# dryajov/zkinterface-ir

Hardware: NVIDIA B200
Metric: field gates evaluated/sec (higher is better)
Workload: dtype u32x8 (255-bit field, Montgomery)

## Files before the change

### zkinterface-ir_b200/csrc/kernels.cu

```cuda
#include <cuda_runtime.h>
#include <stdint.h>
#include <stdlib.h>
#include <string.h>

#include <cooperative_groups.h>

#include "device_util.cuh"
#include "kernels.cuh"

namespace cg = cooperative_groups;

namespace zkb {

template <int N>
__global__ void k_to_mont(uint32_t* consts, uint32_t n, FieldParams fp) {
    uint32_t i = blockIdx.x * blockDim.x + threadIdx.x;
    if (i >= n) return;
    uint32_t a[N], r[N];
#pragma unroll
    for (int k = 0; k < N; k++) a[k] = consts[(size_t)i * N + k];
    fe_mont_mul<N>(r, a, fp.r2, fp.p, fp.n0inv);
#pragma unroll
    for (int k = 0; k < N; k++) consts[(size_t)i * N + k] = r[k];
}
// ... 119 lines not shown
}

template <int N, bool RARE>
__global__ void __launch_bounds__(256)
k_level(const GateOp* __restrict__ ops, const uint32_t* __restrict__ aseq, uint64_t n_ops, uint32_t* __restrict__ store,
        const uint32_t* __restrict__ consts_mont, uint32_t* __restrict__ first_fail, RawCtx rc, TileGeom g, FieldParams fp) {
    const uint64_t total = n_ops << g.log2_wt;
    const uint32_t wt_mask = (1u << g.log2_wt) - 1;
    const bool single = g.log2_wt == 0;
    for (uint64_t tid = blockIdx.x * (uint64_t)blockDim.x + threadIdx.x; tid < total;
         tid += (uint64_t)gridDim.x * blockDim.x) {
        const uint32_t lane = (uint32_t)tid & wt_mask;
        const uint64_t gi = tid >> g.log2_wt;
        const uint4 raw = __ldg(reinterpret_cast<const uint4*>(ops) + gi);
        const uint32_t opc = raw.w & 0xff;
        uint32_t a[N], b[N], r[N];
        load_elem<N>(a, store, raw.x, lane, g.log2_wt);
        if (!RARE) {
            if (opc == D_ADDC || opc == D_MULC) {
#pragma unroll
                for (int k = 0; k < N; k++) b[k] = __ldg(consts_mont + (size_t)raw.y * N + k);
            } else {
                load_elem<N>(b, store, raw.y, lane, g.log2_wt);
            }
            if (opc == D_ADD || opc == D_ADDC) fe_add<N>(r, a, b, fp.p);
            else fe_mont_mul<N>(r, a, b, fp.p, fp.n0inv);
        } else {
            if (opc == D_AND || opc == D_XOR) {
                load_elem<N>(b, store, raw.y, lane, g.log2_wt);
            } else {
#pragma unroll
                for (int k = 0; k < N; k++) b[k] = 0;
            }
            rare_gate<N>(r, a, b, raw, lane, g, rc, fp);
        }
        if (!(raw.w & (F_NOSTORE | g.skip_mask))) store_elem<N>(store, raw.z, lane, g.log2_wt, r);
        if (raw.w & F_ASSERT) {
            bool fail = !fe_is_zero<N>(r) && lane < g.n_valid;
            report_fail(fail, __ldg(aseq + gi), first_fail, g.batch0 + lane, single);
        }
    }
}

template <int N, int LPT>
__device__ __forceinline__ void load_operands(uint32_t* a, uint32_t* b, const uint4& d, const uint32_t* __restrict__ store,
                                              const uint32_t* __restrict__ consts_mont, uint32_t plane, uint32_t log2_pwt) {
    constexpr int PN = N * LPT;
    const uint32_t opc = d.w & 0xff;
    load_elem<PN>(a, store, d.x, plane, log2_pwt);
    if (opc == D_ADDC || opc == D_MULC) {
#pragma unroll
        for (int l = 0; l < LPT; l++)
#pragma unroll
            for (int k = 0; k < N; k++) b[l * N + k] = __ldg(consts_mont + (size_t)d.y * N + k);
    } else {
        load_elem<PN>(b, store, d.y, plane, log2_pwt);
    }
}

#ifndef ZKB_LEVEL_PIPE_MIN_CTAS
#define ZKB_LEVEL_PIPE_MIN_CTAS 4
#endif
template <int N, int LPT>
__global__ void __launch_bounds__(256, ZKB_LEVEL_PIPE_MIN_CTAS)
k_level_pipe(const GateOp* __restrict__ ops, const uint32_t* __restrict__ aseq, uint64_t n_ops, uint32_t* __restrict__ store,
             const uint32_t* __restrict__ consts_mont, uint32_t* __restrict__ first_fail, TileGeom g, FieldParams fp) {
    constexpr int PN = N * LPT;
    constexpr uint32_t kLog2Lpt = LPT == 4 ? 2 : LPT == 2 ? 1 : 0;
    const uint32_t log2_pwt = g.log2_wt - kLog2Lpt;
    const uint64_t total = n_ops << log2_pwt;
    const uint32_t pwt_mask = (1u << log2_pwt) - 1;
    const bool single = g.log2_wt == 0;
    const uint64_t stride = (uint64_t)gridDim.x * blockDim.x;
    uint64_t t0 = blockIdx.x * (uint64_t)blockDim.x + threadIdx.x;
    if (t0 >= total) return;
    const uint4* dptr = reinterpret_cast<const uint4*>(ops);
    uint64_t t1 = t0 + stride, t2 = t1 + stride;
    uint4 d0 = __ldg(dptr + (t0 >> log2_pwt));
    uint4 d1 = t1 < total ? __ldg(dptr + (t1 >> log2_pwt)) : make_uint4(0, 0, 0, 0);
    uint32_t a0[PN], b0[PN], a1[PN], b1[PN];
    load_operands<N, LPT>(a0, b0, d0, store, consts_mont, (uint32_t)t0 & pwt_mask, log2_pwt);
    while (true) {
        uint4 d2 = make_uint4(0, 0, 0, 0);
        if (t2 < total) d2 = __ldg(dptr + (t2 >> log2_pwt));
        const bool more = t1 < total;
        if (more) load_operands<N, LPT>(a1, b1, d1, store, consts_mont, (uint32_t)t1 & pwt_mask, log2_pwt);
        const uint32_t opc = d0.w & 0xff;
        const uint32_t plane = (uint32_t)t0 & pwt_mask;
        uint32_t r[PN];
#pragma unroll
        for (int l = 0; l < LPT; l++) {
            if (opc == D_ADD || opc == D_ADDC) fe_add<N>(r + l * N, a0 + l * N, b0 + l * N, fp.p);
            else fe_mont_mul<N>(r + l * N, a0 + l * N, b0 + l * N, fp.p, fp.n0inv);
        }
        if (!(d0.w & (F_NOSTORE | g.skip_mask))) store_elem<PN>(store, d0.z, plane, log2_pwt, r);
        if (d0.w & F_ASSERT) {
            const uint32_t seq = __ldg(aseq + (t0 >> log2_pwt));
#pragma unroll
            for (int l = 0; l < LPT; l++) {
                const uint32_t lane = plane * LPT + l;
                bool fail = !fe_is_zero<N>(r + l * N) && lane < g.n_valid;
                report_fail(fail, seq, first_fail, g.batch0 + lane, single);
            }
        }
        if (!more) break;
#pragma unroll
        for (int k = 0; k < PN; k++) {
            a0[k] = a1[k];
            b0[k] = b1[k];
        }
        d0 = d1;
        d1 = d2;
        t0 = t1;
        t1 = t2;
        t2 += stride;
    }
}

#ifndef ZKB_TMA_STAGES
#define ZKB_TMA_STAGES 3
#endif
#ifndef ZKB_TMA_MIN_CTAS
#define ZKB_TMA_MIN_CTAS 4
#endif
__device__ __forceinline__ void mbar_init(uint32_t bar, uint32_t count) {
    asm volatile("mbarrier.init.shared::cta.b64 [%0], %1;" ::"r"(bar), "r"(count) : "memory");
}
__device__ __forceinline__ void mbar_expect_tx(uint32_t bar, uint32_t bytes) {
    asm volatile("mbarrier.arrive.expect_tx.shared::cta.b64 _, [%0], %1;" ::"r"(bar), "r"(bytes) : "memory");
}
__device__ __forceinline__ void mbar_wait(uint32_t bar, uint32_t parity) {
    asm volatile(
        "{\n"
        ".reg .pred p;\n"
        "WAIT_%=:\n"
        "mbarrier.try_wait.parity.shared::cta.b64 p, [%0], %1;\n"
        "@p bra DONE_%=;\n"
        "bra WAIT_%=;\n"
        "DONE_%=:\n"
        "}\n" ::"r"(bar), "r"(parity) : "memory");
}
__device__ __forceinline__ void bulk_g2s(uint32_t dst, const void* src, uint32_t bytes, uint32_t bar) {
    asm volatile("cp.async.bulk.shared::cluster.global.mbarrier::complete_tx::bytes [%0], [%1], %2, [%3];" ::"r"(dst), "l"(src), "r"(bytes),
                 "r"(bar)
                 : "memory");
}
__device__ __forceinline__ uint4 lds128(uint32_t a) {
    uint4 v;
    asm volatile("ld.shared.v4.u32 {%0, %1, %2, %3}, [%4];" : "=r"(v.x), "=r"(v.y), "=r"(v.z), "=r"(v.w) : "r"(a));
    return v;
}

constexpr size_t kTmaSmemBytes = (size_t)ZKB_TMA_STAGES * 16384;

template <int N>
__global__ void __launch_bounds__(256, ZKB_TMA_MIN_CTAS)
k_level_tma(const GateOp* __restrict__ ops, const uint32_t* __restrict__ aseq, uint64_t n_ops, uint32_t* __restrict__ store,
            const uint32_t* __restrict__ consts_mont, uint32_t* __restrict__ first_fail, TileGeom g, FieldParams fp) {
    static_assert(N == 8, "two 16-byte chunks per element");
    constexpr int S = ZKB_TMA_STAGES;
    constexpr uint32_t ELEM = 8192, STAGE = 2 * ELEM;
    extern __shared__ __align__(128) uint8_t tma_smem[];
    __shared__ __align__(8) uint64_t full_bar[S];
    const uint32_t smem0 = (uint32_t)__cvta_generic_to_shared(tma_smem);
    const uint32_t bar0 = (uint32_t)__cvta_generic_to_shared(full_bar);
    const uint4* dptr = reinterpret_cast<const uint4*>(ops);
    const uint8_t* store_b = reinterpret_cast<const uint8_t*>(store);
    const uint32_t log2_q = g.log2_wt - 8;
    const uint32_t q_mask = (1u << log2_q) - 1;
    const uint64_t n_items = n_ops << log2_q;
    const uint32_t row = 4096u << log2_q;
    const uint64_t stride = gridDim.x;
    uint64_t gi = blockIdx.x;
    if (gi >= n_items) return;
    auto issue = [&](uint32_t stage, const uint4& d, uint32_t q) {
        const uint32_t opc = d.w & 0xff;
        const bool two = !(opc == D_ADDC || opc == D_MULC);
        const uint32_t bar = bar0 + stage * 8;
        mbar_expect_tx(bar, two ? STAGE : ELEM);
        const uint8_t* pa = store_b + (size_t)d.x * 2 * row + (size_t)q * 4096;
        bulk_g2s(smem0 + stage * STAGE, pa, 4096, bar);
        bulk_g2s(smem0 + stage * STAGE + 4096, pa + row, 4096, bar);
        if (two) {
            const uint8_t* pb = store_b + (size_t)d.y * 2 * row + (size_t)q * 4096;
            bulk_g2s(smem0 + stage * STAGE + ELEM, pb, 4096, bar);
            bulk_g2s(smem0 + stage * STAGE + ELEM + 4096, pb + row, 4096, bar);
        }
    };
    uint64_t gp = gi;
    uint4 dp = make_uint4(0, 0, 0, 0);
    if (threadIdx.x == 0) {
#pragma unroll
        for (int i = 0; i < S; i++) mbar_init(bar0 + i * 8, 1);
        asm volatile("fence.mbarrier_init.release.cluster;" ::: "memory");
        asm volatile("fence.proxy.async.shared::cta;" ::: "memory");
#pragma unroll
        for (int i = 0; i < S; i++) {
            if (gp < n_items) issue(i, __ldg(dptr + (gp >> log2_q)), (uint32_t)gp & q_mask);
            gp += stride;
        }
        if (gp < n_items) dp = __ldg(dptr + (gp >> log2_q));
    }
    __syncthreads();
    uint4 d0 = __ldg(dptr + (gi >> log2_q));
    for (uint32_t it = 0;; it++) {
        const uint64_t gn = gi + stride;
        uint4 d1 = make_uint4(0, 0, 0, 0);
        if (gn < n_items) d1 = __ldg(dptr + (gn >> log2_q));
        const uint32_t lane = (((uint32_t)gi & q_mask) << 8) + threadIdx.x;
        const uint32_t stage = it % S, parity = (it / S) & 1;
        const uint32_t opc = d0.w & 0xff;
        uint32_t a[N], b[N], r[N];
        mbar_wait(bar0 + stage * 8, parity);
        const uint32_t sa = smem0 + stage * STAGE + threadIdx.x * 16;
        unpack(lds128(sa), a);
        unpack(lds128(sa + 4096), a + 4);
        if (opc == D_ADDC || opc == D_MULC) {
#pragma unroll
            for (int k = 0; k < N; k++) b[k] = __ldg(consts_mont + (size_t)d0.y * N + k);
        } else {
            unpack(lds128(sa + ELEM), b);
            unpack(lds128(sa + ELEM + 4096), b + 4);
        }
        __syncthreads();
        if (threadIdx.x == 0) {
            if (gp < n_items) {
                issue(stage, dp, (uint32_t)gp & q_mask);
                gp += stride;
                if (gp < n_items) dp = __ldg(dptr + (gp >> log2_q));
            }
        }
        if (opc == D_ADD || opc == D_ADDC) fe_add<N>(r, a, b, fp.p);
        else fe_mont_mul<N>(r, a, b, fp.p, fp.n0inv);
        if (!(d0.w & (F_NOSTORE | g.skip_mask))) store_elem<N>(store, d0.z, lane, g.log2_wt, r);
        if (d0.w & F_ASSERT) {
            const uint32_t seq = __ldg(aseq + (gi >> log2_q));
            bool fail = !fe_is_zero<N>(r) && lane < g.n_valid;
            report_fail(fail, seq, first_fail, g.batch0 + lane, false);
        }
        if (gn >= n_items) break;
        d0 = d1;
        gi = gn;
    }
}

__device__ __forceinline__ void grid_barrier(uint32_t* ctr, uint32_t target) {
    __syncthreads();
    if (threadIdx.x == 0) {
        asm volatile("red.release.gpu.global.add.u32 [%0], 1;" ::"l"(ctr) : "memory");
        uint32_t v;
        do {
            asm volatile("ld.relaxed.gpu.global.u32 %0, [%1];" : "=r"(v) : "l"(ctr) : "memory");
        } while ((int32_t)(v - target) < 0);
        asm volatile("fence.acq_rel.gpu;" ::: "memory");
    }
    __syncthreads();
}

#ifdef ZKB_COOP_PROFILE
__device__ __forceinline__ long long zkb_clock() {
    long long t;
    asm volatile("mov.u64 %0, %%clock64;" : "=l"(t)::"memory");
    return t;
}
#endif
__device__ __forceinline__ uint4 ldg_pinned(const uint4* p) {
    uint4 v;
    asm volatile("ld.global.nc.v4.u32 {%0, %1, %2, %3}, [%4];" : "=r"(v.x), "=r"(v.y), "=r"(v.z), "=r"(v.w) : "l"(p));
    return v;
}

template <int N, bool CLUSTER>
__global__ void __launch_bounds__(CLUSTER ? 512 : 256)
k_levels_coop(const GateOp* __restrict__ ops, const uint32_t* __restrict__ aseq, const uint64_t* __restrict__ level_off,
              uint32_t n_levels, uint32_t* store, const uint32_t* __restrict__ consts_mont, uint32_t* __restrict__ first_fail,
              RawCtx rc, TileGeom g, FieldParams fp, uint32_t* barrier_ctr, uint32_t barrier_base) {
    const uint32_t wt_mask = (1u << g.log2_wt) - 1;
    const bool single = g.log2_wt == 0;
    const uint64_t stride = (uint64_t)gridDim.x * blockDim.x;
    const uint64_t tid0 = blockIdx.x * (uint64_t)blockDim.x + threadIdx.x;
    const uint4* dptr = reinterpret_cast<const uint4*>(ops);
    constexpr uint32_t kOffCache = 2048;
    __shared__ uint64_t s_off[kOffCache + 1];
    for (uint32_t i = threadIdx.x; i <= n_levels && i <= kOffCache; i += blockDim.x) s_off[i] = level_off[i];
    __syncthreads();
    auto off = [&](uint32_t i) -> uint64_t { return i <= kOffCache ? s_off[i] : level_off[i]; };
    uint64_t lo = off(0), hi = n_levels ? off(1) : lo;
    uint4 first = make_uint4(0, 0, 0, 0);
    if (tid0 < ((hi - lo) << g.log2_wt)) first = ldg_pinned(dptr + lo + (tid0 >> g.log2_wt));
#ifdef ZKB_COOP_PROFILE
    long long prof[7] = {0, 0, 0, 0, 0, 0, 0};
#endif
    for (uint32_t l = 0; l < n_levels; l++) {
#ifdef ZKB_COOP_PROFILE
        const long long th0 = zkb_clock();
#endif
        const uint64_t total = (hi - lo) << g.log2_wt;
        uint64_t nlo = hi, nhi = hi;
        uint4 next_first = make_uint4(0, 0, 0, 0);
        if (l + 1 < n_levels) {
            nhi = off(l + 2);
            if (tid0 < ((nhi - nlo) << g.log2_wt)) next_first = ldg_pinned(dptr + nlo + (tid0 >> g.log2_wt));
        }
#ifdef ZKB_COOP_PROFILE
        const long long tw0 = zkb_clock();
        prof[0] += tw0 - th0;
#endif
        for (uint64_t tid = tid0; tid < total; tid += stride) {
            const uint32_t lane = (uint32_t)tid & wt_mask;
            const uint64_t gi = lo + (tid >> g.log2_wt);
            const uint4 raw = tid == tid0 ? first : __ldg(dptr + gi);
            const uint32_t opc = raw.w & 0xff;
            uint32_t a[N], b[N], r[N];
            load_elem_coherent<N>(a, store, raw.x, lane, g.log2_wt);
            if (opc == D_ADDC || opc == D_MULC) {
#pragma unroll
                for (int k = 0; k < N; k++) b[k] = __ldg(consts_mont + (size_t)raw.y * N + k);
            } else if (opc == D_ADD || opc == D_MUL || opc == D_AND || opc == D_XOR) {
                load_elem_coherent<N>(b, store, raw.y, lane, g.log2_wt);
            } else {
#pragma unroll
                for (int k = 0; k < N; k++) b[k] = 0;
            }
#ifdef ZKB_COOP_PROFILE
            long long tq0 = zkb_clock();
            prof[6] += tq0 - tw0;
            if ((a[0] ^ b[0]) == 0x12345678u) tq0++;
            const long long tq1 = zkb_clock();
            prof[3] += tq1 - tq0;
#endif
            if (opc == D_ADD || opc == D_ADDC) fe_add<N>(r, a, b, fp.p);
            else if (opc == D_MUL || opc == D_MULC) fe_mont_mul<N>(r, a, b, fp.p, fp.n0inv);
            else rare_gate<N>(r, a, b, raw, lane, g, rc, fp);
#ifdef ZKB_COOP_PROFILE
            long long tq2 = zkb_clock();
            if (r[0] == 0x12345679u) tq2++;
            prof[4] += tq2 - tq1;
#endif
            if (!(raw.w & F_NOSTORE)) store_elem<N>(store, raw.z, lane, g.log2_wt, r);
            if (raw.w & F_ASSERT) {
                bool fail = !fe_is_zero<N>(r) && lane < g.n_valid;
                report_fail(fail, __ldg(aseq + gi), first_fail, g.batch0 + lane, single);
            }
#ifdef ZKB_COOP_PROFILE
            prof[5] += zkb_clock() - tq2;
#endif
        }
#ifdef ZKB_COOP_PROFILE
        prof[1] += zkb_clock() - tw0;
#endif
        first = next_first;
        lo = nlo;
        hi = nhi;
        if (l + 1 < n_levels) {
#ifdef ZKB_COOP_PROFILE
            const long long tb0 = zkb_clock();
#endif
            if (CLUSTER) cg::this_cluster().sync();
            else if (barrier_ctr) grid_barrier(barrier_ctr, barrier_base + gridDim.x * (l + 1));
            else cg::this_grid().sync();
#ifdef ZKB_COOP_PROFILE
            prof[2] += zkb_clock() - tb0;
#endif
        }
    }
#ifdef ZKB_COOP_PROFILE
    if ((threadIdx.x & 31) == 0 && (blockIdx.x == 0 || blockIdx.x == gridDim.x - 1) && (threadIdx.x == 0 || threadIdx.x == blockDim.x - 32))
        printf("coop profile cta %u warp %u: levels %u  head %lld  work %lld (issue %lld operands %lld compute %lld store+assert %lld)  barrier %lld  (cycles per level)\n",
               blockIdx.x, threadIdx.x / 32, n_levels, prof[0] / n_levels, prof[1] / n_levels, prof[6] / n_levels, prof[3] / n_levels, prof[4] / n_levels,
               prof[5] / n_levels, prof[2] / n_levels);
#endif
}

template <int N>
__device__ __forceinline__ uint64_t flow_peek(const uint32_t* store, uint32_t slot) {
    if constexpr (N == 2) {
        uint64_t v;
        asm volatile("ld.relaxed.gpu.global.u64 %0, [%1];" : "=l"(v) : "l"(reinterpret_cast<const uint64_t*>(store) + slot) : "memory");
        return v;
    } else {
        uint32_t v;
        asm volatile("ld.relaxed.gpu.global.u32 %0, [%1];" : "=r"(v) : "l"(store + slot) : "memory");
        return v == ~0u ? ~0ull : (uint64_t)v;
    }
}
template <int N>
__device__ __forceinline__ void flow_publish_elem(uint32_t* store, uint32_t slot, const uint32_t* r) {
    if constexpr (N == 2) {
        const uint64_t v = (uint64_t)r[1] << 32 | r[0];
        asm volatile("st.relaxed.gpu.global.u64 [%0], %1;" ::"l"(reinterpret_cast<uint64_t*>(store) + slot), "l"(v) : "memory");
    } else {
        asm volatile("st.relaxed.gpu.global.u32 [%0], %1;" ::"l"(store + slot), "r"(r[0]) : "memory");
    }
}

// ... 443 lines not shown
                } else {
                    uint32_t a[N], one[N], r[N];
                    load_elem<N>(a, store, d.slot, j, g.log2_wt);
#pragma unroll
                    for (int k = 0; k < N; k++) one[k] = (k == 0);
                    fe_mont_mul<N>(r, a, one, fp.p, fp.n0inv);
#pragma unroll
                    for (int k = 0; k < N; k++) dst[k] = r[k];
                    w = N;
                }
            } else {
                const uint8_t* src;
                uint32_t len;
                if (d.kind == CAP_RAW_CONST) {
                    src = raw_consts + (size_t)d.opb * raw_stride;
                    len = raw_stride;
                } else {
                    const uint64_t widx = g.batch0 + j;
                    src = (d.kind == CAP_INSTANCE ? in.inst + widx * in.inst_set_stride : in.wit + widx * in.wit_set_stride) +
                          (uint64_t)d.opb * in.stride;
                    len = in.stride;
                }
                for (; 4 * w < len; w++) {
                    uint32_t x = 0;
                    for (uint32_t b = 0; b < 4 && 4 * w + b < len; b++) x |= (uint32_t)src[4 * w + b] << (8 * b);
                    dst[w] = x;
                }
            }
            for (; w < ew; w++) dst[w] = 0;
        }
        __syncthreads();
        const uint32_t nl = min(kCaptureLanes, g.n_valid - lb * kCaptureLanes);
        const uint32_t per_lane = nv * ew;
        for (uint32_t q = v * kCaptureLanes + l; q < nl * per_lane; q += vb * kCaptureLanes) {
            const uint32_t ll = q / per_lane, r = q - ll * per_lane;
            out[((size_t)(g.batch0 + lb * kCaptureLanes + ll) * n + i0) * ew + r] = cap_sm[ll * row + r];
        }
        __syncthreads();
    }
}

template <int N>
__global__ void __launch_bounds__(256)
k_capture(const CaptureDesc* __restrict__ descs, uint32_t n, const uint32_t* __restrict__ store, InputDesc in,
          const uint8_t* __restrict__ raw_consts, uint32_t raw_stride, TileGeom g, uint32_t ew, uint32_t* __restrict__ out, FieldParams fp) {
    capture_tile<N>(descs, n, store, in, raw_consts, raw_stride, g, ew, out, fp);
}

__global__ void __launch_bounds__(256)
k_bool_capture(const CaptureDesc* __restrict__ descs, uint32_t n, const uint32_t* __restrict__ store, InputDesc in,
               const uint8_t* __restrict__ raw_consts, uint32_t raw_stride, TileGeom g, uint32_t ew, uint32_t* __restrict__ out, FieldParams fp) {
    capture_tile<0>(descs, n, store, in, raw_consts, raw_stride, g, ew, out, fp);
}

__global__ void k_unsink(GateOp* ops, uint64_t n_ops, const uint32_t* __restrict__ slot_bits, uint32_t* found, uint32_t cap, uint32_t* n_found) {
    for (uint64_t i = blockIdx.x * (uint64_t)blockDim.x + threadIdx.x; i < n_ops; i += (uint64_t)gridDim.x * blockDim.x) {
        const uint32_t m = ops[i].meta;
        if (!(m & F_SINK)) continue;
        const uint32_t s = ops[i].out;
        if (!((slot_bits[s >> 5] >> (s & 31)) & 1)) continue;
        ops[i].meta = m & ~F_SINK;
        const uint32_t k = atomicAdd(n_found, 1u);
        if (k < cap) found[k] = (uint32_t)i;
    }
}

__global__ void k_set_sink(GateOp* ops, const uint32_t* __restrict__ idx, uint32_t n, uint32_t set) {
    const uint32_t i = blockIdx.x * blockDim.x + threadIdx.x;
    if (i >= n) return;
    GateOp& op = ops[idx[i]];
    op.meta = set ? (op.meta | F_SINK) : (op.meta & ~F_SINK);
}

__global__ void k_fill_u32(uint32_t* p, uint32_t v, uint64_t n) {
    for (uint64_t i = blockIdx.x * (uint64_t)blockDim.x + threadIdx.x; i < n; i += (uint64_t)gridDim.x * blockDim.x) p[i] = v;
}

static bool level_pipe_enabled() {
    static int v = -1;
    if (v < 0) {
        const char* e = getenv("ZKB_LEVEL_PIPE");
        v = e ? (atoi(e) != 0) : 1;
    }
    return v != 0;
}
static bool level_tma_enabled() {
    const char* e = getenv("ZKB_LEVEL_TMA");
    return e ? atoi(e) != 0 : true;
}
static int grid_per_sm(int dflt) {
    static int v = -1;
    if (v < 0) {
        const char* e = getenv("ZKB_GRID_PER_SM");
        v = e ? atoi(e) : 0;
    }
    return v > 0 ? v : dflt;
}

static inline unsigned grid_for(uint64_t total, int sm_count, int per_sm) {
    uint64_t blocks = (total + 255) / 256;
    uint64_t cap = (uint64_t)sm_count * per_sm;
    if (blocks > cap) blocks = cap;
    if (blocks == 0) blocks = 1;
    return (unsigned)blocks;
}

#define ZKB_DISPATCH_N(nlimb, CALL)         \
    switch (nlimb) {                        \
        case 1: { constexpr int N = 1; CALL; } break; \
        case 2: { constexpr int N = 2; CALL; } break; \
        case 4: { constexpr int N = 4; CALL; } break; \
        default: { constexpr int N = 8; CALL; } break; \
    }

void launch_to_mont(int nlimb, uint32_t* consts, uint32_t n, const FieldParams& fp, cudaStream_t s) {
    if (n == 0) return;
    ZKB_DISPATCH_N(nlimb, (k_to_mont<N><<<(n + 127) / 128, 128, 0, s>>>(consts, n, fp)));
}

void launch_load_inputs(int nlimb, const InputLoad* loads, uint32_t n_loads, uint32_t* store, const uint32_t* consts_mont,
                        InputDesc in, TileGeom g, uint32_t* unreduced_count, uint8_t* rawflag, const uint8_t* const_flags,
                        const FieldParams& fp, int sm_count, cudaStream_t s) {
    if (n_loads == 0) return;
    unsigned grid = grid_for((uint64_t)n_loads << g.log2_wt, sm_count, 256);
    ZKB_DISPATCH_N(nlimb, (k_load_inputs<N><<<grid, 256, 0, s>>>(loads, n_loads, store, consts_mont, in, g, unreduced_count, rawflag,
                                                                 const_flags, fp)));
}

void launch_level(int nlimb, const GateOp* ops, const uint32_t* aseq, uint64_t n_ops, uint32_t* store,
                  const uint32_t* consts_mont, uint32_t* first_fail, const RawCtx& rc, TileGeom g, const FieldParams& fp,
                  int sm_count, bool rare, cudaStream_t s) {
    if (n_ops == 0) return;
    unsigned grid = grid_for(n_ops << g.log2_wt, sm_count, grid_per_sm(256));
    if (!rare) {
        if (level_pipe_enabled()) {
            static const bool pack = getenv("ZKB_LEVEL_LPT") == nullptr || atoi(getenv("ZKB_LEVEL_LPT")) != 1;
            if (pack && nlimb == 2 && g.log2_wt >= 6) {
                grid = grid_for(n_ops << (g.log2_wt - 1), sm_count, grid_per_sm(256));
                k_level_pipe<2, 2><<<grid, 256, 0, s>>>(ops, aseq, n_ops, store, consts_mont, first_fail, g, fp);
            } else if (pack && nlimb == 1 && g.log2_wt >= 7) {
                grid = grid_for(n_ops << (g.log2_wt - 2), sm_count, grid_per_sm(256));
                k_level_pipe<1, 4><<<grid, 256, 0, s>>>(ops, aseq, n_ops, store, consts_mont, first_fail, g, fp);
            } else if (nlimb == 8 && g.log2_wt >= 8 && level_tma_enabled()) {
                static int tma_per_sm = 0;
                static std::atomic<uint64_t> tma_attr_seen{0};
                constexpr size_t smem = kTmaSmemBytes;
                if (first_on_device(tma_attr_seen))
                    cudaFuncSetAttribute(k_level_tma<8>, cudaFuncAttributeMaxDynamicSharedMemorySize, (int)smem);
                if (!tma_per_sm) {
                    const char* e = getenv("ZKB_TMA_GRID_PER_SM");
                    tma_per_sm = e ? std::max(1, atoi(e)) : 128;
                }
                grid = grid_for(n_ops << g.log2_wt, sm_count, tma_per_sm);
                k_level_tma<8><<<grid, 256, smem, s>>>(ops, aseq, n_ops, store, consts_mont, first_fail, g, fp);
            } else {
                ZKB_DISPATCH_N(nlimb, (k_level_pipe<N, 1><<<grid, 256, 0, s>>>(ops, aseq, n_ops, store, consts_mont, first_fail, g, fp)));
            }
        } else {
            ZKB_DISPATCH_N(nlimb, (k_level<N, false><<<grid, 256, 0, s>>>(ops, aseq, n_ops, store, consts_mont, first_fail, rc, g, fp)));
        }
    } else {
        ZKB_DISPATCH_N(nlimb, (k_level<N, true><<<grid, 256, 0, s>>>(ops, aseq, n_ops, store, consts_mont, first_fail, rc, g, fp)));
    }
}

template <int N>
static cudaError_t launch_coop_n(const GateOp* ops, const uint32_t* aseq, const uint64_t* level_off, uint32_t n_levels, uint32_t* store,
                                 const uint32_t* consts_mont, uint32_t* first_fail, RawCtx rc, TileGeom g, FieldParams fp,
                                 int sm_count, uint64_t max_level_items, uint32_t* barrier_ctr, uint32_t* barrier_epoch, cudaStream_t s) {
    static const bool counter_barrier = getenv("ZKB_COUNTER_BARRIER") != nullptr;
    if (!counter_barrier) barrier_ctr = nullptr;
    uint32_t barrier_base = *barrier_epoch;
    void* args[] = {(void*)&ops, (void*)&aseq, (void*)&level_off, (void*)&n_levels, (void*)&store, (void*)&consts_mont,
                    (void*)&first_fail, (void*)&rc, (void*)&g, (void*)&fp, (void*)&barrier_ctr, (void*)&barrier_base};
    static const bool no_cluster = getenv("ZKB_NO_CLUSTER") != nullptr;
    static bool cluster_ok = true;
    if (!no_cluster && cluster_ok && max_level_items <= 8 * 512 * 2) {
        cudaLaunchConfig_t cfg = {};
        cfg.gridDim = dim3(8);
        cfg.blockDim = dim3(512);
        cfg.stream = s;
        cudaLaunchAttribute attr[1];
        attr[0].id = cudaLaunchAttributeClusterDimension;
        attr[0].val.clusterDim.x = 8;
        attr[0].val.clusterDim.y = 1;
        attr[0].val.clusterDim.z = 1;
        cfg.attrs = attr;
        cfg.numAttrs = 1;
        cudaError_t ec = cudaLaunchKernelExC(&cfg, (const void*)k_levels_coop<N, true>, args);
        if (ec == cudaSuccess) return ec;
        cudaGetLastError();
        cluster_ok = false;
    }
    int per_sm = 0;
    cudaError_t e = cudaOccupancyMaxActiveBlocksPerMultiprocessor(&per_sm, k_levels_coop<N, false>, 256, 0);
    if (e != cudaSuccess) return e;
    if (per_sm < 1) return cudaErrorLaunchOutOfResources;
    uint64_t want = (max_level_items + 255) / 256;
    uint64_t blocks = ((want + sm_count - 1) / sm_count) * sm_count;
    if (blocks < (uint64_t)sm_count) blocks = sm_count;
    if (blocks > (uint64_t)sm_count * per_sm) blocks = (uint64_t)sm_count * per_sm;
    if (const char* e = getenv("ZKB_COOP_BLOCKS")) blocks = (uint64_t)atoi(e);
    e = cudaLaunchCooperativeKernel((void*)k_levels_coop<N, false>, dim3((unsigned)blocks), dim3(256), args, 0, s);
    if (e == cudaSuccess && barrier_ctr && n_levels > 1) *barrier_epoch += (uint32_t)blocks * (n_levels - 1);
    return e;
}

template <int KIND>
__global__ void __launch_bounds__(KIND == 2 ? 512 : 256) k_barrier_only(uint32_t n, uint32_t* ctr, uint32_t base, uint32_t* sink) {
    uint32_t acc = 0;
    for (uint32_t i = 0; i < n; i++) {
        if (KIND == 0) cg::this_grid().sync();
        else if (KIND == 1) grid_barrier(ctr, base + gridDim.x * (i + 1));
        else cg::this_cluster().sync();
        acc += i;
    }
    if (acc == 0xFFFFFFFFu) *sink = acc;
}

cudaError_t measure_barrier_cost(int kind, unsigned blocks, unsigned n_barriers, uint32_t* barrier_ctr, uint32_t* barrier_epoch,
                                 cudaStream_t s, cudaEvent_t ev0, cudaEvent_t ev1, float* us_per_barrier) {
    uint32_t base = *barrier_epoch;
    uint32_t* sink = barrier_ctr;
    float best = 1e30f;
    for (int rep = 0; rep < 4; rep++) {
        float ms[2] = {0, 0};
        for (int pass = 0; pass < 2; pass++) {
            uint32_t n = pass == 0 ? 0u : n_barriers;
            base = *barrier_epoch;
            void* args[] = {(void*)&n, (void*)&barrier_ctr, (void*)&base, (void*)&sink};
            cudaEventRecord(ev0, s);
            cudaError_t e;
            if (kind == 2) {
                cudaLaunchConfig_t cfg = {};
                cfg.gridDim = dim3(8);
                cfg.blockDim = dim3(512);
                cfg.stream = s;
                cudaLaunchAttribute attr[1];
                attr[0].id = cudaLaunchAttributeClusterDimension;
                attr[0].val.clusterDim.x = 8;
                attr[0].val.clusterDim.y = 1;
                attr[0].val.clusterDim.z = 1;
                cfg.attrs = attr;
                cfg.numAttrs = 1;
                e = cudaLaunchKernelExC(&cfg, (const void*)k_barrier_only<2>, args);
            } else if (kind == 1) {
                e = cudaLaunchCooperativeKernel((void*)k_barrier_only<1>, dim3(blocks), dim3(256), args, 0, s);
                if (e == cudaSuccess) *barrier_epoch += blocks * n;
            } else {
                e = cudaLaunchCooperativeKernel((void*)k_barrier_only<0>, dim3(blocks), dim3(256), args, 0, s);
            }
            if (e != cudaSuccess) return e;
            cudaEventRecord(ev1, s);
            e = cudaStreamSynchronize(s);
            if (e != cudaSuccess) return e;
            cudaEventElapsedTime(&ms[pass], ev0, ev1);
        }
        if (rep > 0) best = std::min(best, ms[1] - ms[0]);
    }
    *us_per_barrier = best * 1e3f / (float)n_barriers;
    return cudaSuccess;
}

cudaError_t launch_levels_coop(int nlimb, const GateOp* ops, const uint32_t* aseq, const uint64_t* level_off, uint32_t n_levels,
                               uint32_t* store, const uint32_t* consts_mont, uint32_t* first_fail, const RawCtx& rc, TileGeom g,
                               const FieldParams& fp, int sm_count, uint64_t max_level_items, uint32_t* barrier_ctr,
                               uint32_t* barrier_epoch, cudaStream_t s) {
    cudaError_t e = cudaSuccess;
    ZKB_DISPATCH_N(nlimb, (e = launch_coop_n<N>(ops, aseq, level_off, n_levels, store, consts_mont, first_fail, rc, g, fp, sm_count,
                                                max_level_items, barrier_ctr, barrier_epoch, s)));
    return e;
}

template <int N>
static cudaError_t launch_flow_n(const GateOp* ops, const uint32_t* aseq, const uint64_t* level_off, uint32_t n_levels, uint32_t* store,
                                 const uint32_t* consts_mont, uint32_t* first_fail, RawCtx rc, TileGeom g, FieldParams fp, int sm_count,
                                 uint64_t max_level_items, uint32_t fill_from, uint32_t n_slots, cudaStream_t s) {
    int per_sm = 0;
    cudaError_t e = cudaOccupancyMaxActiveBlocksPerMultiprocessor(&per_sm, k_levels_flow<N>, 256, 0);
    if (e != cudaSuccess) return e;
    if (per_sm < 1) return cudaErrorLaunchOutOfResources;
    uint64_t want = (max_level_items + 255) / 256;
    uint64_t blocks = ((want + sm_count - 1) / sm_count) * sm_count;
    if (blocks < (uint64_t)sm_count) blocks = sm_count;
    if (blocks > (uint64_t)sm_count * per_sm) blocks = (uint64_t)sm_count * per_sm;
    if (const char* eb = getenv("ZKB_FLOW_BLOCKS")) blocks = std::min<uint64_t>((uint64_t)std::max(1, atoi(eb)), (uint64_t)sm_count * per_sm);
    if (n_slots > fill_from) {
        e = cudaMemsetAsync(store + (size_t)fill_from * N, 0xFF, (size_t)(n_slots - fill_from) * N * 4, s);
        if (e != cudaSuccess) return e;
    }
    uint32_t sleep_ns = 0;
    if (const char* es = getenv("ZKB_FLOW_SLEEP")) sleep_ns = (uint32_t)atoi(es);
    void* args[] = {(void*)&ops, (void*)&aseq, (void*)&level_off, (void*)&n_levels, (void*)&store, (void*)&consts_mont,
                    (void*)&first_fail, (void*)&rc, (void*)&g, (void*)&fp, (void*)&sleep_ns};
    return cudaLaunchCooperativeKernel((void*)k_levels_flow<N>, dim3((unsigned)blocks), dim3(256), args, 0, s);
}
template <int N>
static cudaError_t launch_flow_wide_n(const GateOp* ops, const uint32_t* aseq, const uint64_t* level_off, uint32_t n_levels, uint32_t* store,
                                      const uint32_t* consts_mont, uint32_t* first_fail, RawCtx rc, TileGeom g, FieldParams fp, int sm_count,
                                      uint64_t max_level_items, uint32_t n_ready, uint32_t* flags, uint32_t epoch, cudaStream_t s) {
    int per_sm = 0;
    cudaError_t e = cudaOccupancyMaxActiveBlocksPerMultiprocessor(&per_sm, k_levels_flow_wide<N>, 256, 0);
    if (e != cudaSuccess) return e;
    if (per_sm < 1) return cudaErrorLaunchOutOfResources;
    uint64_t want = (max_level_items + 255) / 256;
    uint64_t blocks = ((want + sm_count - 1) / sm_count) * sm_count;
    if (blocks < (uint64_t)sm_count) blocks = sm_count;
// ... 167 lines not shown
```

Before: 77.92 billion.

## Add dedicated producer warp with empty/full mbarriers to TMA level kernel

Restructures the TMA level kernel into a warp-specialized producer/consumer pipeline: an extra warp issues bulk copies and writes op descriptors to shared memory, and consumer warps signal per-stage empty barriers instead of a block-wide __syncthreads. This removes the per-iteration block barrier and lets the refill overlap with compute. It costs an extra warp per CTA, which may cut occupancy under the launch bounds, and adds barrier traffic.

```diff
diff --git a/zkinterface-ir_b200/csrc/kernels.cu b/zkinterface-ir_b200/csrc/kernels.cu
--- a/zkinterface-ir_b200/csrc/kernels.cu
+++ b/zkinterface-ir_b200/csrc/kernels.cu
@@ -295,18 +295,28 @@
 }
 
 constexpr size_t kTmaSmemBytes = (size_t)ZKB_TMA_STAGES * 16384;
-
-template <int N>
-__global__ void __launch_bounds__(256, ZKB_TMA_MIN_CTAS)
+constexpr int kTmaThreads = 256 + 32;
+__device__ __forceinline__ void mbar_arrive(uint32_t bar) {
+    asm volatile("mbarrier.arrive.shared::cta.b64 _, [%0];" ::"r"(bar) : "memory");
+}
+__device__ __forceinline__ void sts128(uint32_t a, const uint4& v) {
+    asm volatile("st.shared.v4.u32 [%0], {%1, %2, %3, %4};" ::"r"(a), "r"(v.x), "r"(v.y), "r"(v.z), "r"(v.w) : "memory");
+}
+
+template <int N>
+__global__ void __launch_bounds__(kTmaThreads, ZKB_TMA_MIN_CTAS)
 k_level_tma(const GateOp* __restrict__ ops, const uint32_t* __restrict__ aseq, uint64_t n_ops, uint32_t* __restrict__ store,
             const uint32_t* __restrict__ consts_mont, uint32_t* __restrict__ first_fail, TileGeom g, FieldParams fp) {
     static_assert(N == 8, "two 16-byte chunks per element");
     constexpr int S = ZKB_TMA_STAGES;
     constexpr uint32_t ELEM = 8192, STAGE = 2 * ELEM;
     extern __shared__ __align__(128) uint8_t tma_smem[];
-    __shared__ __align__(8) uint64_t full_bar[S];
+    __shared__ __align__(8) uint64_t full_bar[S], empty_bar[S];
+    __shared__ __align__(16) uint4 desc[S];
     const uint32_t smem0 = (uint32_t)__cvta_generic_to_shared(tma_smem);
-    const uint32_t bar0 = (uint32_t)__cvta_generic_to_shared(full_bar);
+    const uint32_t full0 = (uint32_t)__cvta_generic_to_shared(full_bar);
+    const uint32_t empty0 = (uint32_t)__cvta_generic_to_shared(empty_bar);
+    const uint32_t desc0 = (uint32_t)__cvta_generic_to_shared(desc);
     const uint4* dptr = reinterpret_cast<const uint4*>(ops);
     const uint8_t* store_b = reinterpret_cast<const uint8_t*>(store);
     const uint32_t log2_q = g.log2_wt - 8;
@@ -314,64 +324,66 @@
     const uint64_t n_items = n_ops << log2_q;
     const uint32_t row = 4096u << log2_q;
     const uint64_t stride = gridDim.x;
-    uint64_t gi = blockIdx.x;
-    if (gi >= n_items) return;
-    auto issue = [&](uint32_t stage, const uint4& d, uint32_t q) {
-        const uint32_t opc = d.w & 0xff;
-        const bool two = !(opc == D_ADDC || opc == D_MULC);
-        const uint32_t bar = bar0 + stage * 8;
-        mbar_expect_tx(bar, two ? STAGE : ELEM);
-        const uint8_t* pa = store_b + (size_t)d.x * 2 * row + (size_t)q * 4096;
-        bulk_g2s(smem0 + stage * STAGE, pa, 4096, bar);
-        bulk_g2s(smem0 + stage * STAGE + 4096, pa + row, 4096, bar);
-        if (two) {
-            const uint8_t* pb = store_b + (size_t)d.y * 2 * row + (size_t)q * 4096;
-            bulk_g2s(smem0 + stage * STAGE + ELEM, pb, 4096, bar);
-            bulk_g2s(smem0 + stage * STAGE + ELEM + 4096, pb + row, 4096, bar);
-        }
-    };
-    uint64_t gp = gi;
-    uint4 dp = make_uint4(0, 0, 0, 0);
+    if (blockIdx.x >= n_items) return;
     if (threadIdx.x == 0) {
 #pragma unroll
-        for (int i = 0; i < S; i++) mbar_init(bar0 + i * 8, 1);
+        for (int i = 0; i < S; i++) {
+            mbar_init(full0 + i * 8, 1);
+            mbar_init(empty0 + i * 8, 256 / 32);
+        }
         asm volatile("fence.mbarrier_init.release.cluster;" ::: "memory");
         asm volatile("fence.proxy.async.shared::cta;" ::: "memory");
-#pragma unroll
-        for (int i = 0; i < S; i++) {
-            if (gp < n_items) issue(i, __ldg(dptr + (gp >> log2_q)), (uint32_t)gp & q_mask);
-            gp += stride;
-        }
-        if (gp < n_items) dp = __ldg(dptr + (gp >> log2_q));
     }
     __syncthreads();
-    uint4 d0 = __ldg(dptr + (gi >> log2_q));
-    for (uint32_t it = 0;; it++) {
-        const uint64_t gn = gi + stride;
-        uint4 d1 = make_uint4(0, 0, 0, 0);
-        if (gn < n_items) d1 = __ldg(dptr + (gn >> log2_q));
+    if (threadIdx.x >= 256) {
+        if (threadIdx.x != 256) return;
+        uint64_t gp = blockIdx.x;
+        uint4 dp = __ldg(dptr + (gp >> log2_q));
+        for (uint32_t it = 0;; it++) {
+            const uint32_t stage = it % S;
+            const uint64_t gn = gp + stride;
+            uint4 dn = make_uint4(0, 0, 0, 0);
+            if (gn < n_items) dn = __ldg(dptr + (gn >> log2_q));
+            if (it >= S) mbar_wait(empty0 + stage * 8, (it / S - 1) & 1);
+            sts128(desc0 + stage * 16, dp);
+            const uint32_t opc = dp.w & 0xff;
+            const bool two = !(opc == D_ADDC || opc == D_MULC);
+            const uint32_t bar = full0 + stage * 8;
+            const uint32_t q = (uint32_t)gp & q_mask;
+            mbar_expect_tx(bar, two ? STAGE : ELEM);
+            const uint8_t* pa = store_b + (size_t)dp.x * 2 * row + (size_t)q * 4096;
+            bulk_g2s(smem0 + stage * STAGE, pa, 4096, bar);
+            bulk_g2s(smem0 + stage * STAGE + 4096, pa + row, 4096, bar);
+            if (two) {
+                const uint8_t* pb = store_b + (size_t)dp.y * 2 * row + (size_t)q * 4096;
+                bulk_g2s(smem0 + stage * STAGE + ELEM, pb, 4096, bar);
+                bulk_g2s(smem0 + stage * STAGE + ELEM + 4096, pb + row, 4096, bar);
+            }
+            if (gn >= n_items) return;
+            dp = dn;
+            gp = gn;
+        }
+    }
+    for (uint64_t gi = blockIdx.x, it = 0; gi < n_items; gi += stride, it++) {
+        const uint32_t stage = (uint32_t)(it % S), parity = (uint32_t)(it / S) & 1;
         const uint32_t lane = (((uint32_t)gi & q_mask) << 8) + threadIdx.x;
-        const uint32_t stage = it % S, parity = (it / S) & 1;
+        uint32_t a[N], b[N], r[N];
+        mbar_wait(full0 + stage * 8, parity);
+        const uint4 d0 = lds128(desc0 + stage * 16);
         const uint32_t opc = d0.w & 0xff;
-        uint32_t a[N], b[N], r[N];
-        mbar_wait(bar0 + stage * 8, parity);
         const uint32_t sa = smem0 + stage * STAGE + threadIdx.x * 16;
         unpack(lds128(sa), a);
         unpack(lds128(sa + 4096), a + 4);
-        if (opc == D_ADDC || opc == D_MULC) {
-#pragma unroll
-            for (int k = 0; k < N; k++) b[k] = __ldg(consts_mont + (size_t)d0.y * N + k);
-        } else {
+        const bool konst = opc == D_ADDC || opc == D_MULC;
+        if (!konst) {
             unpack(lds128(sa + ELEM), b);
             unpack(lds128(sa + ELEM + 4096), b + 4);
         }
-        __syncthreads();
-        if (threadIdx.x == 0) {
-            if (gp < n_items) {
-                issue(stage, dp, (uint32_t)gp & q_mask);
-                gp += stride;
-                if (gp < n_items) dp = __ldg(dptr + (gp >> log2_q));
-            }
+        __syncwarp();
+        if ((threadIdx.x & 31) == 0) mbar_arrive(empty0 + stage * 8);
+        if (konst) {
+#pragma unroll
+            for (int k = 0; k < N; k++) b[k] = __ldg(consts_mont + (size_t)d0.y * N + k);
         }
         if (opc == D_ADD || opc == D_ADDC) fe_add<N>(r, a, b, fp.p);
         else fe_mont_mul<N>(r, a, b, fp.p, fp.n0inv);
@@ -381,9 +393,6 @@
             bool fail = !fe_is_zero<N>(r) && lane < g.n_valid;
             report_fail(fail, seq, first_fail, g.batch0 + lane, false);
         }
-        if (gn >= n_items) break;
-        d0 = d1;
-        gi = gn;
     }
 }
 
@@ -1133,7 +1142,7 @@
                     tma_per_sm = e ? std::max(1, atoi(e)) : 128;
                 }
                 grid = grid_for(n_ops << g.log2_wt, sm_count, tma_per_sm);
-                k_level_tma<8><<<grid, 256, smem, s>>>(ops, aseq, n_ops, store, consts_mont, first_fail, g, fp);
+                k_level_tma<8><<<grid, kTmaThreads, smem, s>>>(ops, aseq, n_ops, store, consts_mont, first_fail, g, fp);
             } else {
                 ZKB_DISPATCH_N(nlimb, (k_level_pipe<N, 1><<<grid, 256, 0, s>>>(ops, aseq, n_ops, store, consts_mont, first_fail, g, fp)));
             }
```

Result: faster. 81.44 billion, median of 6 (+4.5%).
